# cockroachdb/pebble

Measured on AMD Instinct MI355X. Metric: raw-block GiB/s decoded to KV arrays (device-resident), 1/2/4/8 MI355X, higher is better.
Workload: dtype u8; 1 GPU; config2: 65536 x 32 KiB row-format blocks per GPU, restart interval 16, 16 B keys / 100 B values; blocks_per_gpu=65536, input_bytes_per_gpu=2143748096, kvs_per_gpu=17760256, global_batch_blocks=65536, parallelism=shard1

## Files before the change

### pebble_amd/csrc/common.hip.h

```cpp
#pragma once
#include <hip/hip_runtime.h>
#include <stdint.h>

#include <type_traits>

#include "../../include/pebble_amd.h"

namespace pbl {

typedef uint32_t u32x4 __attribute__((ext_vector_type(4)));
typedef uint32_t u32x2 __attribute__((ext_vector_type(2)));

constexpr int kTPB = 256;
constexpr int kWave = 64;
constexpr int kNumComp = 4;
#ifndef PBL_LB_WIN
#define PBL_LB_WIN 2
#endif
constexpr int kLbWin = PBL_LB_WIN;
#ifndef PBL_LB_L2
#define PBL_LB_L2 0
#endif
constexpr bool kLbL2 = PBL_LB_L2 != 0;

constexpr uint64_t kKindInvalidTrailer = 191u;

__device__ __forceinline__ uint64_t with_seq(uint64_t tr, uint64_t seq, uint32_t flags) {
  return (seq && !(flags & PBL_ROW_RAW_KEYS) && tr != kKindInvalidTrailer) ? (seq << 8) | (tr & 0xff) : tr;
}

constexpr uint64_t kWsHeader = 256;
constexpr int kWsColTick = 2;
constexpr int kWsRowCount = 3;
constexpr uint32_t kSplitChunk = 4096;
constexpr int kStShift = 61;
constexpr uint64_t kStAgg = 1ull << kStShift;
constexpr uint64_t kStWide = 2ull << kStShift;
constexpr uint64_t kStPfx = 3ull << kStShift;
constexpr uint64_t kStPfxWide = 4ull << kStShift;
constexpr uint64_t kStMask = 7ull << kStShift;
constexpr uint64_t kValMask = (1ull << kStShift) - 1;
constexpr int kPkBits[kNumComp] = {14, 18, 18, 11};
constexpr int kPkShift[kNumComp] = {0, 14, 32, 50};
constexpr int kPfBits[kNumComp] = {31, 30, 37, 24};

constexpr uint32_t kL2Chunk = 64;
__host__ __device__ inline uint64_t ws_l2_offset(uint32_t n_blocks) {
  return kWsHeader + uint64_t(2 + 2 * kNumComp) * n_blocks * 8ull;
}
__host__ __device__ inline uint64_t ws_bytes(uint32_t n_blocks) {
  return ws_l2_offset(n_blocks) + 16ull * ((uint64_t(n_blocks) + kL2Chunk - 1) / kL2Chunk);
}
__host__ __device__ inline uint64_t ws_rcnt_offset(uint32_t n_blocks) {
  return ws_l2_offset(n_blocks) - 8ull * (n_blocks + 1);
}
#ifdef PBL_STAMPS
constexpr uint64_t kStampWords = 16;
#else
constexpr uint64_t kStampWords = 0;
#endif
__host__ __device__ inline uint64_t ws_ids_offset(uint32_t n_blocks) {
  return ws_bytes(n_blocks) + kStampWords * 8ull * n_blocks;
}
__host__ __device__ inline uint64_t ws_redo_offset(uint32_t n_blocks) {
  return ws_ids_offset(n_blocks) + 4ull * n_blocks + 4ull * (n_blocks / kSplitChunk + 1) + 8;
}
__host__ __device__ inline uint64_t ws_pend_offset(uint32_t n_blocks) { return ws_redo_offset(n_blocks) + 4ull * n_blocks; }
constexpr uint32_t kEntRec = 64;
__host__ __device__ inline uint64_t ws_ent_offset(uint32_t n_blocks) {
  return (ws_pend_offset(n_blocks) + 4ull * n_blocks + 15) & ~uint64_t(15);
}
__host__ __device__ inline uint64_t ws_alloc_bytes(uint32_t n_blocks) {
  return ws_ent_offset(n_blocks) + 2ull * kEntRec * n_blocks;
}
constexpr uint32_t kLongKeyWgs = PBL_LONGKEY_WGS;
__host__ __device__ inline uint64_t ws_spill_slot_bytes(uint64_t workspace_bytes, uint32_t n_blocks) {
  const uint64_t a = ws_alloc_bytes(n_blocks);
  return workspace_bytes > a ? ((workspace_bytes - a) / kLongKeyWgs) & ~uint64_t(15) : 0;
}


template <class T>
using gptr = __attribute__((address_space(1))) T*;
template <class T>
using lptr = __attribute__((address_space(3))) T*;
template <class T>
__device__ __forceinline__ gptr<T> to_glb(T* p) {
  return (gptr<T>)p;
}
template <class T>
__device__ __forceinline__ lptr<T> to_lds_ptr(T* p) {
  return (lptr<T>)p;
}

__device__ inline uint32_t g_atomic_add(uint32_t* p, uint32_t v) {
  return __hip_atomic_fetch_add(to_glb(p), v, __ATOMIC_RELAXED, __HIP_MEMORY_SCOPE_AGENT);
}
__device__ inline uint32_t g_atomic_or(uint32_t* p, uint32_t v) {
  return __hip_atomic_fetch_or(to_glb(p), v, __ATOMIC_RELAXED, __HIP_MEMORY_SCOPE_AGENT);
}

struct TicketQueue {
  uint32_t* tick;
  uint32_t n_blocks;
  __device__ uint32_t take() const {
    const uint32_t t = g_atomic_add(tick, 1u);
    return t < n_blocks ? t : n_blocks;
  }
};
struct ListQueue {
  uint32_t* tick;
  const uint32_t* ids;
  uint32_t n;
  uint32_t n_blocks;
  __device__ uint32_t take() const {
    const uint32_t t = g_atomic_add(tick, 1u);
    return t < n ? to_glb(ids)[t] : n_blocks;
  }
};

__device__ inline uint64_t ld_agent(const uint64_t* p) {
  return __hip_atomic_load(to_glb(p), __ATOMIC_RELAXED, __HIP_MEMORY_SCOPE_AGENT);
}
__device__ inline void st_agent(uint64_t* p, uint64_t v) {
  __hip_atomic_store(to_glb(p), v, __ATOMIC_RELAXED, __HIP_MEMORY_SCOPE_AGENT);
}

__device__ inline int lane_id() { return threadIdx.x & (kWave - 1); }
__device__ inline int wave_id() { return threadIdx.x >> 6; }

__device__ inline void wave_sync() {
  __builtin_amdgcn_fence(__ATOMIC_RELEASE, "wavefront");
  __builtin_amdgcn_wave_barrier();
  __builtin_amdgcn_fence(__ATOMIC_ACQUIRE, "wavefront");
}

template <typename T>
__device__ inline T wave_incl_scan(T v) {
  const int l = lane_id();
#pragma unroll
  for (int d = 1; d < kWave; d <<= 1) {
    T o = __shfl_up(v, d, kWave);
    if (l >= d) v += o;
  }
  return v;
}
template <typename T>
__device__ inline T wave_sum(T v) {
#pragma unroll
  for (int d = 32; d >= 1; d >>= 1) v += __shfl_xor(v, d, kWave);
  return v;
}

__device__ inline void block_excl_scan2(uint32_t a, uint32_t b, uint32_t* ea, uint32_t* eb,
                                        uint32_t* scratch, uint32_t* tot_a, uint32_t* tot_b) {
  uint32_t ia = wave_incl_scan(a), ib = wave_incl_scan(b);
  const int w = wave_id(), l = lane_id();
  if (l == kWave - 1) { scratch[w] = ia; scratch[4 + w] = ib; }
  __syncthreads();
  uint32_t pa = 0, pb = 0, ta = 0, tb = 0;
#pragma unroll
  for (int i = 0; i < kTPB / kWave; i++) {
    uint32_t sa = scratch[i], sb = scratch[4 + i];
    if (i < w) { pa += sa; pb += sb; }
    ta += sa; tb += sb;
  }
  *ea = pa + ia - a;
  *eb = pb + ib - b;
  *tot_a = ta;
  *tot_b = tb;
}

__device__ inline void lds_stage16(lptr<u32x4> dst, gptr<const u32x4> src, uint32_t n16) {
  const uint32_t l = lane_id();
  for (uint32_t g0 = 0; g0 < n16; g0 += kWave) {
    if (g0 + l < n16)
      __builtin_amdgcn_global_load_lds((gptr<const void>)(src + (g0 + l)), (lptr<void>)(dst + g0), 16, 0, 0);
  }
  asm volatile("s_waitcnt vmcnt(0)" ::: "memory");
  wave_sync();
}

__device__ inline bool agg_packable(const uint64_t agg[kNumComp]) {
  return agg[0] < (1ull << kPkBits[0]) && agg[1] < (1ull << kPkBits[1]) && agg[2] < (1ull << kPkBits[2]) &&
         agg[3] < (1ull << kPkBits[3]);
}
__device__ inline bool pfx_packable(const uint64_t p[kNumComp]) {
  return p[0] < (1ull << kPfBits[0]) && p[1] < (1ull << kPfBits[1]) && p[2] < (1ull << kPfBits[2]) &&
         p[3] < (1ull << kPfBits[3]);
}

struct LbPtrs {
  uint64_t* rec;
  uint64_t* pfx;
  uint64_t* wide;
  uint64_t* l2;
  __device__ LbPtrs(uint64_t* st, uint32_t n_blocks)
      : rec(st), pfx(st + 2ull * n_blocks), wide(st + 2ull * n_blocks + uint64_t(kNumComp) * n_blocks),
        l2(st + (ws_l2_offset(n_blocks) - kWsHeader) / 8) {}
};

__device__ inline void l2_store(const LbPtrs& P, uint32_t chunk, uint64_t tag, const uint64_t p[kNumComp]) {
  st_agent(P.l2 + 2ull * chunk + 1, tag | p[2] | (p[3] << kPfBits[2]));
  st_agent(P.l2 + 2ull * chunk, tag | p[0] | (p[1] << kPfBits[0]));
}

#ifdef PBL_STAMPS
struct LbDiag {
  uint32_t trips, recs, recs2;
  uint64_t poll;
};
#define LBDIAG(...) __VA_ARGS__
#else
struct LbDiag {};
#define LBDIAG(...)
#endif

__device__ inline void lb_store_pfx(const LbPtrs& P, uint32_t n_blocks, uint32_t v, const uint64_t p[kNumComp]) {
  const int l = lane_id();
  if (pfx_packable(p)) {
    if (l == 0) {
      st_agent(P.rec + 2ull * v + 1, kStPfx | p[2] | (p[3] << kPfBits[2]));
      st_agent(P.rec + 2ull * v, kStPfx | p[0] | (p[1] << kPfBits[0]));
    }
  } else {
    if (l < kNumComp) {
      const uint64_t x = l == 0 ? p[0] : l == 1 ? p[1] : l == 2 ? p[2] : p[3];
      st_agent(P.pfx + uint64_t(l) * n_blocks + v, kStPfxWide | (x & kValMask));
    }
    if (l == 0) st_agent(P.rec + 2ull * v, kStPfxWide);
  }
}

__device__ inline void lb_publish(uint64_t* st, uint32_t n_blocks, uint32_t v, const uint64_t agg[kNumComp]) {
  const int l = lane_id();
  const LbPtrs P(st, n_blocks);
  if (v == 0) {
    lb_store_pfx(P, n_blocks, v, agg);
    return;
  }
  if (agg_packable(agg)) {
    if (l == 0) {
      uint64_t packed = 0;
      for (int c = 0; c < kNumComp; c++) packed |= agg[c] << kPkShift[c];
      st_agent(P.rec + 2ull * v, kStAgg | packed);
    }
  } else {
    if (l < kNumComp) {
      const uint64_t a = l == 0 ? agg[0] : l == 1 ? agg[1] : l == 2 ? agg[2] : agg[3];
      st_agent(P.wide + uint64_t(l) * n_blocks + v, kStWide | (a & kValMask));
    }
    if (l == 0) st_agent(P.rec + 2ull * v, kStWide);
  }
}

__device__ inline uint64_t lb_poll(uint64_t* p, uint64_t want, uint32_t* spins, bool* timed_out) {
  uint64_t x;
  while (((x = ld_agent(p)) & kStMask) != want) {
    if (++*spins > (1u << 22)) { *timed_out = true; return 0; }
    __builtin_amdgcn_s_sleep(2);
  }
  return x & kValMask;
}

__device__ inline void lb_fetch4(uint64_t* src, uint32_t n_blocks, int64_t idx, uint64_t want, uint64_t c[kNumComp],
                                 uint32_t* spins, bool* timed_out) {
  uint64_t x[kNumComp];
#pragma unroll
  for (int q = 0; q < kNumComp; q++) x[q] = ld_agent(src + uint64_t(q) * n_blocks + idx);
#pragma unroll
  for (int q = 0; q < kNumComp; q++)
    c[q] = (x[q] & kStMask) == want ? (x[q] & kValMask)
                                    : lb_poll(src + uint64_t(q) * n_blocks + idx, want, spins, timed_out);
}

template <bool L2>
struct LbChunkWin {};
template <>
struct LbChunkWin<true> {
  uint64_t c0, c1;
};
template <int W, bool L2 = false>
struct LbWindows : LbChunkWin<L2> {
  static_assert(!L2 || W >= 2, "two windows reach the chunk edge");
  uint64_t w0[W], w1[W];
  int64_t top;
  __device__ inline int64_t chunk() const { return (top + 1) >> 6; }
  __device__ inline void issue(const LbPtrs& P, int64_t top_) {
    top = top_;
    const int l = lane_id();
    int64_t lo = 0;
    if constexpr (L2) lo = chunk() >= 1 ? (chunk() - 1) * int64_t(kL2Chunk) : 0;
#pragma unroll
    for (int k = 0; k < W; k++) {
      const int64_t idx = top - kWave * k - l;
      const bool in = idx >= lo;
      w0[k] = in ? ld_agent(P.rec + 2 * idx) : idx < 0 ? kStPfx : kStAgg;
      w1[k] = in ? ld_agent(P.rec + 2 * idx + 1) : kStPfx;
    }
    if constexpr (L2) {
      const int64_t c = chunk() - 2 - l;
      this->c0 = c >= 0 ? ld_agent(P.l2 + 2 * c) : kStPfx;
      this->c1 = c >= 0 ? ld_agent(P.l2 + 2 * c + 1) : kStPfx;
    }
  }
};

template <int W, bool L2>
__device__ inline bool lb_consume(const LbPtrs& P, uint32_t n_blocks, const LbWindows<W, L2>& G, uint64_t acc[kNumComp],
                                  int64_t* next_top, int64_t* wait_idx, uint32_t* spins, bool* timed_out, LbDiag* D) {
  const int l = lane_id();
  int64_t top = G.top;
  *wait_idx = -1;
#pragma unroll
  for (int k = 0; k < W; k++) {
    const int64_t idx = G.top - kWave * k - l;
    const uint64_t state = G.w0[k] & kStMask;
    const bool is_pfx = state == kStPfx || state == kStPfxWide;
    const uint64_t pfxm = __ballot(is_pfx);
    const uint64_t notready = __ballot(state == 0);
    const int first = pfxm ? __builtin_ctzll(pfxm) : 64;
    const uint64_t need = first >= 63 ? ~0ull : ((2ull << first) - 1);
    if (notready & need) {
      *wait_idx = G.top - kWave * k - __builtin_ctzll(notready & need);
      *next_top = top;
      return false;
    }
    LBDIAG(D->recs += __builtin_popcountll(__ballot(l <= first && idx >= 0 && (G.w0[k] != kStAgg))));
    uint64_t c[kNumComp] = {0, 0, 0, 0};
    if (l < first && state == kStAgg) {
#pragma unroll
      for (int q = 0; q < kNumComp; q++) c[q] = (G.w0[k] >> kPkShift[q]) & ((1ull << kPkBits[q]) - 1);
    }
    if (l < first && state == kStWide) lb_fetch4(P.wide, n_blocks, idx, kStWide, c, spins, timed_out);
    if (l == first && idx >= 0) {
      if (state == kStPfx) {
        uint64_t w1 = G.w1[k];
        if ((w1 & kStMask) != kStPfx) w1 = kStPfx | lb_poll(P.rec + 2 * idx + 1, kStPfx, spins, timed_out);
        c[0] = G.w0[k] & ((1ull << kPfBits[0]) - 1);
        c[1] = (G.w0[k] >> kPfBits[0]) & ((1ull << kPfBits[1]) - 1);
        c[2] = w1 & ((1ull << kPfBits[2]) - 1);
        c[3] = (w1 >> kPfBits[2]) & ((1ull << kPfBits[3]) - 1);
      } else {
        lb_fetch4(P.pfx, n_blocks, idx, kStPfxWide, c, spins, timed_out);
      }
    }
#pragma unroll
    for (int q = 0; q < kNumComp; q++) acc[q] += c[q];
    if (first < 64) return true;
    top -= kWave;
  }
  if constexpr (L2) {
    const int64_t ck = G.chunk();
    if (ck >= 2) {
      const uint64_t s0 = G.c0 & kStMask, s1 = G.c1 & kStMask;
      const bool there = s0 == s1 && (s0 == kStAgg || s0 == kStPfx);
      const uint64_t pfxm = __ballot(there && s0 == kStPfx), absent = __ballot(!there);
      const int firstp = pfxm ? __builtin_ctzll(pfxm) : 64, firsta = absent ? __builtin_ctzll(absent) : 64;
      const bool ends = firstp < firsta;
      if (ends ? l <= firstp : l < firsta) {
        acc[0] += G.c0 & ((1ull << kPfBits[0]) - 1);
        acc[1] += (G.c0 >> kPfBits[0]) & ((1ull << kPfBits[1]) - 1);
        acc[2] += G.c1 & ((1ull << kPfBits[2]) - 1);
        acc[3] += (G.c1 >> kPfBits[2]) & ((1ull << kPfBits[3]) - 1);
      }
      LBDIAG(D->recs2 += ends ? firstp + (ck - 2 - firstp >= 0) : firsta);
      if (ends) return true;
      top = (ck - 2 - firsta) * int64_t(kL2Chunk) + (kL2Chunk - 1);
    }
  }
  *next_top = top;
  return false;
}

template <int W, bool L2, int WL = W>
__device__ inline void lb_finish(uint64_t* st, uint32_t n_blocks, uint32_t v, const uint64_t agg[kNumComp],
                                 uint64_t excl[kNumComp], uint32_t* timeout_flag, const LbWindows<W, L2>& first_win,
                                 LbDiag* D = nullptr) {
  const int l = lane_id();
  const LbPtrs P(st, n_blocks);
  uint64_t acc[kNumComp] = {0, 0, 0, 0};
  uint32_t spins = 0;
  bool timed_out = false;
  int64_t top = int64_t(v) - 1, wait_idx = -1;
  LBDIAG(LbDiag d0{0, 0, 0, 0}; if (!D) D = &d0; D->trips = v > 0; D->recs = D->recs2 = 0; D->poll = 0);
  if constexpr (L2) {
    if ((v & (kL2Chunk - 1)) == kL2Chunk - 1 && agg_packable(agg)) {
      const uint64_t w = first_win.w0[0];
      if (!__ballot(l < int(kL2Chunk) - 1 && (w & kStMask) != kStAgg)) {
        const uint64_t m = l < int(kL2Chunk) - 1 ? w : 0;
        uint64_t s01 = ((m >> kPkShift[0]) & ((1ull << kPkBits[0]) - 1)) | ((m >> kPkShift[1]) & ((1ull << kPkBits[1]) - 1)) << 32;
        uint64_t s23 = ((m >> kPkShift[2]) & ((1ull << kPkBits[2]) - 1)) | ((m >> kPkShift[3]) & ((1ull << kPkBits[3]) - 1)) << 32;
        s01 = wave_sum(s01);
        s23 = wave_sum(s23);
        const uint64_t ca[kNumComp] = {(s01 & 0xffffffffu) + agg[0], (s01 >> 32) + agg[1], (s23 & 0xffffffffu) + agg[2],
                                       (s23 >> 32) + agg[3]};
        if (l == 0) l2_store(P, v / kL2Chunk, kStAgg, ca);
      }
    }
  }
  bool done = v == 0 || lb_consume(P, n_blocks, first_win, acc, &top, &wait_idx, &spins, &timed_out, D);
  if (__ballot(timed_out)) timed_out = true;
  while (!done && !timed_out) {
    if (wait_idx >= 0) {
      LBDIAG(const uint64_t tp = __builtin_amdgcn_s_memtime());
      if (l == 0) {
        while ((ld_agent(P.rec + 2 * wait_idx) & kStMask) == 0) {
          if (++spins > (1u << 22)) { timed_out = true; break; }
          __builtin_amdgcn_s_sleep(2);
        }
      }
      if (__shfl(timed_out ? 1 : 0, 0, kWave)) { timed_out = true; break; }
      LBDIAG(D->poll += __builtin_amdgcn_s_memtime() - tp);
    }
    LbWindows<WL, L2> G;
    G.issue(P, top);
    LBDIAG(D->trips++);
    done = lb_consume(P, n_blocks, G, acc, &top, &wait_idx, &spins, &timed_out, D);
    if (__ballot(timed_out)) timed_out = true;
  }
  if (timed_out && l == 0) g_atomic_or(timeout_flag, 1u << PBL_TIMEOUT);
#pragma unroll
  for (int q = 0; q < kNumComp; q++) excl[q] = wave_sum(acc[q]);
  if (v > 0) {
    uint64_t p[kNumComp];
#pragma unroll
    for (int q = 0; q < kNumComp; q++) p[q] = excl[q] + agg[q];
    lb_store_pfx(P, n_blocks, v, p);
    if constexpr (L2) {
      if ((v & (kL2Chunk - 1)) == kL2Chunk - 1 && !timed_out && pfx_packable(p) && l == 0)
        l2_store(P, v / kL2Chunk, kStPfx, p);
    }
  }
}

template <int W = kLbWin, bool L2 = false>
__device__ inline void lb_resolve(uint64_t* st, uint32_t n_blocks, uint32_t v, const uint64_t agg[kNumComp],
                                  uint64_t excl[kNumComp], uint32_t* timeout_flag) {
  LbWindows<W, L2> G;
  if (v > 0) G.issue(LbPtrs(st, n_blocks), int64_t(v) - 1);
  lb_finish(st, n_blocks, v, agg, excl, timeout_flag, G);
}

template <bool L2 = false>
__device__ inline void lookback(uint64_t* st, uint32_t n_blocks, uint32_t v, const uint64_t agg[kNumComp],
                                uint64_t excl[kNumComp], uint32_t* timeout_flag) {
  lb_publish(st, n_blocks, v, agg);
  lb_resolve<kLbWin, L2>(st, n_blocks, v, agg, excl, timeout_flag);
}

struct Args {
  pbl_block_batch in;
  pbl_decode_out out;
};

__device__ __forceinline__ uint4 funnel16(const uint4& x, const uint4& y, uint32_t sh) {
  const uint32_t s = sh & 3;
  uint32_t d0, d1, d2, d3, d4;
  switch (sh >> 2) {
    case 0: d0 = x.x; d1 = x.y; d2 = x.z; d3 = x.w; d4 = y.x; break;
    case 1: d0 = x.y; d1 = x.z; d2 = x.w; d3 = y.x; d4 = y.y; break;
    case 2: d0 = x.z; d1 = x.w; d2 = y.x; d3 = y.y; d4 = y.z; break;
    default: d0 = x.w; d1 = y.x; d2 = y.y; d3 = y.z; d4 = y.w; break;
  }
  return make_uint4(__builtin_amdgcn_alignbyte(d1, d0, s), __builtin_amdgcn_alignbyte(d2, d1, s),
                    __builtin_amdgcn_alignbyte(d3, d2, s), __builtin_amdgcn_alignbyte(d4, d3, s));
}

#ifndef PBL_STORE16_NT
#define PBL_STORE16_NT 1
#endif
__device__ inline void store16(uint8_t* base_, uint64_t ga, uint64_t lo, uint64_t hi, uint4 w) {
  const gptr<uint8_t> base = to_glb(base_);
  if (ga >= lo && ga + 16 <= hi) {
#if PBL_STORE16_NT
    __builtin_nontemporal_store(u32x4{w.x, w.y, w.z, w.w}, (gptr<u32x4>)(base + ga));
#else
    *(gptr<u32x4>)(base + ga) = u32x4{w.x, w.y, w.z, w.w};
#endif
    return;
  }
#pragma unroll
  for (int i = 0; i < 16; i++) {
    uint32_t word = i < 4 ? w.x : i < 8 ? w.y : i < 12 ? w.z : w.w;
    if (ga + i >= lo && ga + i < hi) base[ga + i] = uint8_t(word >> (8 * (i & 3)));
  }
}

typedef u32x4 u32x4_u __attribute__((aligned(1)));
typedef uint64_t u64_u __attribute__((aligned(1)));
typedef uint32_t u32_u __attribute__((aligned(1)));
typedef uint16_t u16_u __attribute__((aligned(1)));
__device__ __forceinline__ void copy_chunks(gptr<uint8_t> dst, gptr<const uint8_t> src, uint32_t n) {
  uint32_t c = 0;
  for (; c + 64 <= n; c += 64) {
    u32x4 x[4];
#pragma unroll
    for (int u = 0; u < 4; u++) x[u] = *(gptr<const u32x4_u>)(src + c + 16 * u);
#pragma unroll
    for (int u = 0; u < 4; u++) *(gptr<u32x4_u>)(dst + c + 16 * u) = x[u];
  }
  for (; c + 16 <= n; c += 16) *(gptr<u32x4_u>)(dst + c) = *(gptr<const u32x4_u>)(src + c);
  if (c < n) {
    const u32x4 w = *(gptr<const u32x4_u>)(src + c);
    const uint32_t r = n - c;
    uint64_t lo = uint64_t(w.x) | uint64_t(w.y) << 32, hi = uint64_t(w.z) | uint64_t(w.w) << 32;
    uint32_t o = c;
    if (r & 8) {
      *(gptr<u64_u>)(dst + o) = lo;
      lo = hi;
      o += 8;
    }
    if (r & 4) {
      *(gptr<u32_u>)(dst + o) = uint32_t(lo);
      lo >>= 32;
      o += 4;
    }
    if (r & 2) {
      *(gptr<u16_u>)(dst + o) = uint16_t(lo);
      lo >>= 16;
      o += 2;
    }
    if (r & 1) dst[o] = uint8_t(lo);
  }
}

__device__ inline void write_block_meta(const pbl_decode_out& O, uint32_t b, uint32_t nb, uint32_t status,
                                        const uint64_t excl[kNumComp], const uint64_t agg[kNumComp],
                                        bool slow) {
  to_glb(O.blk_kv_base)[b] = excl[0];
  to_glb(O.blk_key_base)[b] = excl[1];
// ... 39 lines not shown
```

### pebble_amd/csrc/rowblk_pool.hip.h

```cpp
#pragma once

#include "rowblk_core.hip.h"
#include "rowblk_general.hip.h"
#include "rowblk_big.hip.h"

namespace pbl {
namespace row {
namespace pool {

#ifndef PBL_POOL_WAVES
#define PBL_POOL_WAVES 8
#endif
#ifndef PBL_POOL_STAGES
#define PBL_POOL_STAGES 3
#endif
#ifndef PBL_POOL_SLEEP
#define PBL_POOL_SLEEP 8
#endif
#ifndef PBL_POOL_PRIO
#define PBL_POOL_PRIO 2
#endif
#ifndef PBL_POOL_EARLYREL
#define PBL_POOL_EARLYREL 2
#endif
#ifndef PBL_POOL_PREFETCH
#define PBL_POOL_PREFETCH 0
#endif
#ifndef PBL_POOL_PREFETCH_LATE
#define PBL_POOL_PREFETCH_LATE 1
#endif
#ifndef PBL_POOL_LB_WIN
#define PBL_POOL_LB_WIN PBL_LB_WIN
#endif
#ifndef PBL_POOL_LB_WIN_LATER
#define PBL_POOL_LB_WIN_LATER 1
#endif
constexpr int kPoolLbWin = PBL_POOL_LB_WIN;
constexpr int kPoolLbWinLater = kLbL2 ? kPoolLbWin : PBL_POOL_LB_WIN_LATER;
constexpr int kEarlyRel = PBL_POOL_EARLYREL;
constexpr uint32_t kPrefetch = PBL_POOL_PREFETCH;
constexpr int kNW = PBL_POOL_WAVES;
constexpr int kNS = PBL_POOL_STAGES;
constexpr int kTPBP = kNW * kWave;
constexpr uint32_t kMaxKl = 4095;

struct Stage {
  uint4 x[kLdsBlkBytes / 16];
};

__device__ __forceinline__ uint32_t m_ksrc(uint64_t m) { return uint32_t(m) & 0x7fffu; }
__device__ __forceinline__ uint32_t m_sh(uint64_t m) { return uint32_t(m >> 15) & 0xfffu; }
__device__ __forceinline__ uint32_t m_klen(uint64_t m) { return uint32_t(m >> 27) & 0xfffu; }
__device__ __forceinline__ uint32_t m_par(uint64_t m) { return uint32_t(m >> 39) & 0x1ffu; }
__device__ __forceinline__ uint32_t m_hl(uint64_t m) { return uint32_t(m >> 48) & 0xfu; }
__device__ __forceinline__ uint32_t m_fl(uint64_t m) { return uint32_t(m >> 52) & 0xffu; }
__device__ __forceinline__ uint64_t m_pack(uint32_t ksrc, uint32_t sh, uint32_t kl, uint32_t par, uint32_t hl,
                                           uint32_t fl) {
  return uint64_t(ksrc) | uint64_t(sh) << 15 | uint64_t(kl) << 27 | uint64_t(par) << 39 | uint64_t(hl) << 48 |
         uint64_t(fl) << 52;
}

constexpr int kPerSlot = (163840 - kNS * int(sizeof(Stage)) - 256) / kNW;
template <bool kHide>
constexpr int slot_kv() {
  const int n = ((kPerSlot - 32) / (kHide ? 14 : 12)) & ~7;
  return n > 511 ? 511 : n;
}
template <bool kHide>
struct Slot {
  static constexpr int kKv = slot_kv<kHide>();
  uint64_t m0[kKv];
  uint32_t vp[kKv + 5];
  uint16_t ent[kHide ? kKv : 1];
};

template <bool kHide>
struct PoolLds {
  Stage st[kNS];
  Slot<kHide> sl[kNW];
  uint32_t free_mask;
};
static_assert(sizeof(PoolLds<true>) <= 163840 && sizeof(PoolLds<false>) <= 163840, "one pool workgroup per CU");

typedef u32x4 u32x4_ug __attribute__((aligned(1)));
typedef uint32_t u32_ug __attribute__((aligned(1)));
typedef uint64_t u64_ug __attribute__((aligned(1)));
typedef uint16_t u16_ug __attribute__((aligned(1)));

__device__ __forceinline__ uint32_t dpp_incl_scan(uint32_t v) {
  v += __builtin_amdgcn_update_dpp(0u, v, 0x111, 0xf, 0xf, false);
  v += __builtin_amdgcn_update_dpp(0u, v, 0x112, 0xf, 0xf, false);
  v += __builtin_amdgcn_update_dpp(0u, v, 0x114, 0xf, 0xf, false);
  v += __builtin_amdgcn_update_dpp(0u, v, 0x118, 0xf, 0xf, false);
  v += __builtin_amdgcn_update_dpp(0u, v, 0x142, 0xa, 0xf, false);
  v += __builtin_amdgcn_update_dpp(0u, v, 0x143, 0xc, 0xf, false);
  return v;
}
__device__ __forceinline__ uint32_t last_lane(uint32_t v) { return __builtin_amdgcn_readlane(v, kWave - 1); }

#ifndef PBL_POOL_NT
#define PBL_POOL_NT 1
#endif
template <class T>
__device__ __forceinline__ void st_out(gptr<T> p, T v) {
#if PBL_POOL_NT
  __builtin_nontemporal_store(v, p);
#else
  *p = v;
#endif
}

#ifndef PBL_POOL_SBASE
#define PBL_POOL_SBASE 0
#endif
#ifndef PBL_POOL_VFAST
#define PBL_POOL_VFAST 1
#endif
constexpr bool kSBase = PBL_POOL_SBASE != 0;
constexpr bool kVFast = PBL_POOL_VFAST != 0;
// ... 767 lines not shown
      }
    }
  }
}

template <bool kHide>
__device__ __forceinline__ uint32_t acquire(PoolLds<kHide>& L) {
  uint32_t s = 0;
  if (lane_id() == 0) {
    for (;;) {
      const uint32_t m = __hip_atomic_load(&L.free_mask, __ATOMIC_RELAXED, __HIP_MEMORY_SCOPE_WORKGROUP);
      if (m) {
        const uint32_t c = uint32_t(__builtin_ctz(m));
        const uint32_t old =
            __hip_atomic_fetch_and(&L.free_mask, ~(1u << c), __ATOMIC_ACQUIRE, __HIP_MEMORY_SCOPE_WORKGROUP);
        if (old & (1u << c)) {
          s = c;
          break;
        }
      } else {
        __builtin_amdgcn_s_sleep(PBL_POOL_SLEEP);
      }
    }
  }
  if (PBL_POOL_PRIO) __builtin_amdgcn_s_setprio(PBL_POOL_PRIO);
  return __builtin_amdgcn_readfirstlane(__shfl(s, 0, kWave));
}

template <bool kHide>
__device__ __forceinline__ int32_t try_acquire(PoolLds<kHide>& L) {
  int32_t s = -1;
  if (lane_id() == 0) {
    const uint32_t m = __hip_atomic_load(&L.free_mask, __ATOMIC_RELAXED, __HIP_MEMORY_SCOPE_WORKGROUP);
    if (m) {
      const uint32_t c = uint32_t(__builtin_ctz(m));
      const uint32_t old =
          __hip_atomic_fetch_and(&L.free_mask, ~(1u << c), __ATOMIC_ACQUIRE, __HIP_MEMORY_SCOPE_WORKGROUP);
      if (old & (1u << c)) s = int32_t(c);
    }
  }
  return __builtin_amdgcn_readfirstlane(__shfl(s, 0, kWave));
}

template <bool kHide>
__device__ __forceinline__ void release(PoolLds<kHide>& L, uint32_t s, bool drop_prio = true) {
  asm volatile("s_waitcnt lgkmcnt(0)" ::: "memory");
  wave_sync();
  if (lane_id() == 0) __hip_atomic_fetch_or(&L.free_mask, 1u << s, __ATOMIC_RELEASE, __HIP_MEMORY_SCOPE_WORKGROUP);
  if (PBL_POOL_PRIO && drop_prio) __builtin_amdgcn_s_setprio(0);
}

__device__ __forceinline__ void stage_dma(Stage& S, const uint8_t* blocks, uint64_t boff, uint32_t blen) {
  const int l = lane_id();
  const uint64_t a0 = boff & ~uint64_t(15), a1 = (boff + blen + 15) & ~uint64_t(15);
  const uint32_t n16 = uint32_t((a1 - a0) >> 4);
  const gptr<const uint8_t> base = to_glb(blocks + a0);
  for (uint32_t g0 = 0; g0 < n16; g0 += kWave) {
    if (g0 + l < n16)
      __builtin_amdgcn_global_load_lds((gptr<const void>)(base + 16ull * (g0 + l)),
                                       (lptr<void>)to_lds_ptr(reinterpret_cast<void*>(&S.x[1 + g0])), 16, 0, 0);
  }
}

__device__ __noinline__ void block_slow(Stage& S, uint8_t* keybuf, uint32_t keycap, const Args A, uint32_t b,
                                        uint64_t boff, uint32_t blen) {
  const int l = lane_id();
  const uint32_t nb = A.in.n_blocks, flags = A.in.flags;
  const pbl_decode_out& O = A.out;
  uint64_t* lb_state = reinterpret_cast<uint64_t*>(reinterpret_cast<uint8_t*>(O.workspace) + kWsHeader);
  SlowState ss;
  uint64_t dummy[kNumComp] = {0, 0, 0, 0}, excl[kNumComp];
  const uint8_t* src = reinterpret_cast<const uint8_t*>(S.x) + kPad + (boff & 15);
  bool from_lds = true;
  slow_walk(src, true, blen, flags, A.in.synthetic_seq_num, keybuf, keycap, kPassCount, O, b, dummy, &ss);
  if (ss.status == PBL_UNSUPPORTED) {
    from_lds = false;
    src = A.in.blocks + boff;
    keybuf = reinterpret_cast<uint8_t*>(S.x);
    keycap = uint32_t(kLdsBlkBytes);
    slow_walk(src, false, blen, flags, A.in.synthetic_seq_num, keybuf, keycap, kPassCount, O, b, dummy, &ss);
  }
  const bool okk = ss.status == PBL_OK;
  const uint64_t agg[kNumComp] = {okk ? ss.nkv : 0, okk ? ss.kb : 0, okk ? ss.vb : 0, okk ? ss.nr : 0};
  lookback<kLbL2>(lb_state, nb, b, agg, excl, &O.totals->status_mask);
  uint32_t st2 = ss.status;
  if (okk && overflows(O, excl, agg)) st2 = PBL_OVERFLOW;
  if (st2 == PBL_OK) slow_walk(src, from_lds, blen, flags, A.in.synthetic_seq_num, keybuf, keycap, kPassAll, O, b, excl, &ss);
  else if (l == 0 && O.key_off && excl[0] + b < O.kv_cap + nb) {
    to_glb(O.key_off)[excl[0] + b] = 0;
    to_glb(O.val_off)[excl[0] + b] = 0;
  }
  if (l == 0) write_block_meta(O, b, nb, st2, excl, agg, true);
}

__device__ __noinline__ void block_big(const Args A, uint32_t b, uint64_t boff, uint32_t blen, uint8_t* keybuf,
                                       uint32_t keycap) {
  const int l = lane_id();
  const uint32_t nb = A.in.n_blocks;
  const pbl_decode_out& O = A.out;
  uint64_t* lb_state = reinterpret_cast<uint64_t*>(reinterpret_cast<uint8_t*>(O.workspace) + kWsHeader);
  const uint32_t st0 = to_glb(O.blk_status)[b];
  const bool okk = st0 == PBL_OK;
  const uint64_t agg[kNumComp] = {okk ? to_glb(O.blk_kv_base)[b] : 0, okk ? to_glb(O.blk_key_base)[b] : 0,
                                  okk ? to_glb(O.blk_val_base)[b] : 0,
                                  okk ? uint64_t(GlbBlk{to_glb(A.in.blocks + boff), blen}.le32(blen - 4)) : 0};
  uint64_t excl[kNumComp];
  lb_resolve<kLbWin, kLbL2>(lb_state, nb, b, agg, excl, &O.totals->status_mask);
  uint32_t st2 = st0;
  if (okk && overflows(O, excl, agg)) st2 = PBL_OVERFLOW;
  if (l == 0) {
    if (st2 != PBL_OK && O.key_off && excl[0] + b < O.kv_cap + nb) {
      to_glb(O.key_off)[excl[0] + b] = 0;
      to_glb(O.val_off)[excl[0] + b] = 0;
    }
    write_block_meta(O, b, nb, st2, excl, agg, true);
  }
  if (st2 == PBL_OK) {
    SlowState ss;
    slow_walk_t<GlbBlk, PBL_BIG_U>(GlbBlk{to_glb(A.in.blocks + boff), blen}, blen, A.in.flags,
                                    A.in.synthetic_seq_num, to_lds_ptr(keybuf), keycap, kPassAll, O, b, excl, &ss);
    if (ss.status == PBL_UNSUPPORTED && l == 0) {
      uint32_t* hdr = reinterpret_cast<uint32_t*>(O.workspace);
      uint32_t* pend = reinterpret_cast<uint32_t*>(reinterpret_cast<uint8_t*>(O.workspace) + ws_pend_offset(nb));
      to_glb(pend)[g_atomic_add(hdr + rowc::kWsBigPend, 1u)] = b;
    } else if (ss.status != PBL_OK && l == 0) {
      to_glb(O.blk_status)[b] = ss.status;
      g_atomic_or(&O.totals->status_mask, 1u << ss.status);
      g_atomic_add(&O.totals->n_bad_blocks, 1u);
    }
  }
}

struct Pend {
  uint64_t boff;
  uint32_t b, status, nkv, tkb, tvb, nres, roff, blen;
  bool live;
};

template <bool kHide>
__device__ __forceinline__ Pend block_front(PoolLds<kHide>& L, uint32_t s, uint32_t b, uint64_t boff, uint32_t blen,
                                            bool staged, Slot<kHide>& W, const Args& A) {
  Stage& S = L.st[s];
  const int l = lane_id();
  const uint32_t nb = A.in.n_blocks, flags = A.in.flags;
  const bool vprefix = (flags & PBL_ROW_VALUE_PREFIX) && !(flags & PBL_ROW_RAW_KEYS);
  uint64_t* lb_state = reinterpret_cast<uint64_t*>(reinterpret_cast<uint8_t*>(A.out.workspace) + kWsHeader);
  constexpr uint32_t kKv = uint32_t(Slot<kHide>::kKv);
  Pend P;
  P.b = b;
  P.boff = boff;
  P.blen = blen;
  P.live = false;
  P.nkv = P.tkb = P.tvb = P.nres = P.roff = 0;
  P.status = PBL_OK;

  if (blen > kMaxFastLen) {
    release(L, s);
    block_big(A, b, boff, blen, reinterpret_cast<uint8_t*>(&W), uint32_t(sizeof(W)));
    return P;
  }
  PSTAMP(A, b, 1, l == 0);
  if (!staged) stage_dma(S, A.in.blocks, boff, blen);
  asm volatile("s_waitcnt vmcnt(0)" ::: "memory");
  wave_sync();
  PSTAMP(A, b, 2, l == 0);
  const View V = lds_view(S.x, uint32_t(kPad + (boff & 15)));
  uint32_t roff, nres;
  uint32_t status = init_checks(LdsBlk{V}, blen, flags, &roff, &nres);
  bool slow = status == PBL_OK && nres > kKv;
  uint32_t nkv = 0, tkb = 0, tvb = 0;
  bool published = false, released = false;
  if (status == PBL_OK && !slow && roff > 0) {
    const uint32_t R = (nres + kWave - 1) / kWave;
    const uint32_t r0 = min(uint32_t(l) * R, nres), r1 = min(r0 + R, nres);
    PAcc acc{0, 0, 0, 0};
    bool ok = true, bad = false, vbad = false, over = false;
    PRun RB;
    RB.n = 0;
    RB.pos = RB.e0 = RB.prev_kl = RB.prev_kind = RB.rw = 0;
    const bool single = R == 1;
    walk_runs<kHide>(V, r0, r1, nres, roff, flags, vprefix, single, RB, acc, ok, bad, vbad, over);
    const uint32_t ic = dpp_incl_scan(acc.cnt), ik = dpp_incl_scan(acc.kb), iv = dpp_incl_scan(acc.vb);
    const uint32_t ie = kHide ? dpp_incl_scan(acc.ne) : ic;
    nkv = last_lane(ic);
    tkb = last_lane(ik);
    tvb = last_lane(iv);
    const uint32_t nent = kHide ? last_lane(ie) : nkv;
    if (__ballot(bad)) status = PBL_CORRUPT_BOUNDS;
    else if (__ballot(!ok) || nent > kKv) slow = true;
    else if (__ballot(vbad)) status = PBL_CORRUPT_BOUNDS;
// ... 4 lines not shown
      PSTAMP(A, b, 3, l == 0);
      if (kEarlyRel && single && !vprefix && !__ballot(over)) {
        release(L, s, kEarlyRel != 2);
        released = true;
        PSTAMP(A, b, 9, l == 0);
      }
      MState M{ie - (kHide ? acc.ne : acc.cnt), ic - acc.cnt, iv - acc.vb, 0, 0, 0};
      meta_runs<kHide>(W, V, r0, r1, nres, roff, flags, vprefix, single, over, RB, M);
      if (l < 5) W.vp[nkv + l] = tvb;
      PSTAMP(A, b, 4, l == 0);
    }
  }
  if (status == PBL_OK && slow) {
    block_slow(S, reinterpret_cast<uint8_t*>(W.m0), uint32_t(sizeof(W.m0)), A, b, boff, blen);
    release(L, s);
    PSTAMP(A, b, 9, l == 0);
    return P;
  }
  if (!released) {
    release(L, s);
    PSTAMP(A, b, 9, l == 0);
  } else if (PBL_POOL_PRIO && kEarlyRel == 2) {
    __builtin_amdgcn_s_setprio(0);
  }
  if (!published) {
    const bool okb = status == PBL_OK;
    const uint64_t agg[kNumComp] = {okb ? nkv : 0, okb ? tkb : 0, okb ? tvb : 0, okb ? nres : 0};
    lb_publish(lb_state, nb, b, agg);
    if (l < 5) W.vp[l] = 0;
  }
  P.status = status;
  P.nkv = status == PBL_OK ? nkv : 0;
  P.tkb = status == PBL_OK ? tkb : 0;
  P.tvb = status == PBL_OK ? tvb : 0;
  P.nres = status == PBL_OK ? nres : 0;
  P.roff = roff;
  P.live = true;
  return P;
}

struct Next {
  uint32_t t, w;
};
constexpr uint32_t kNextHave = 4, kNextStaged = 8, kNextDone = 16;
static_assert(kNS <= 4, "Next::w keeps the stage in two bits");

template <bool kHide>
__device__ __forceinline__ void prefetch(PoolLds<kHide>& L, const Args& A, const uint32_t* ids, uint32_t nt, Next& X) {
  const int32_t s = try_acquire(L);
  if (s < 0) return;
  uint32_t t = 0;
  if (lane_id() == 0) t = g_atomic_add(reinterpret_cast<uint32_t*>(A.out.workspace), 1u);
  t = __builtin_amdgcn_readfirstlane(__shfl(t, 0, kWave));
  if (t >= nt) {
    release(L, uint32_t(s));
    X.w = kNextDone;
    return;
  }
  if (ids) t = __builtin_amdgcn_readfirstlane(to_glb(ids)[t]);
  const uint64_t boff = to_glb(A.in.block_off)[t];
  const uint32_t blen = to_glb(A.in.block_len)[t];
  const bool staged = blen <= kMaxFastLen;
  X.t = t;
  X.w = uint32_t(s) | kNextHave | (staged ? kNextStaged : 0u);
  if (staged) stage_dma(L.st[s], A.in.blocks, boff, blen);
  PSTAMP(A, t, 10, lane_id() == 0);
}

template <bool kHide>
__device__ __forceinline__ void block_emit(const Pend& P, const Slot<kHide>& W, const Args& A, PoolLds<kHide>& L,
                                           const uint32_t* ids, uint32_t nt, Next& X) {
  const int l = lane_id();
  const uint32_t nb = A.in.n_blocks, flags = A.in.flags, b = P.b;
  const pbl_decode_out& O = A.out;
  uint64_t* lb_state = reinterpret_cast<uint64_t*>(reinterpret_cast<uint8_t*>(O.workspace) + kWsHeader);
  const uint8_t* gblk = A.in.blocks + P.boff;
  const gptr<const uint8_t> gb = ubase<kSBase>(to_glb(gblk));
  const uint32_t ph = uint32_t(uint64_t(gblk) & 15u);
  const gptr<const uint8_t> g16 = ubase<kSBase>(to_glb(gblk - ph));
  constexpr bool kFastSteps = kVFast && kUni && kVDepth == 1;
  const GSrc KS{gb, P.blen, uint32_t(((uint64_t(gblk) + P.blen + 15) & ~uint64_t(15)) - uint64_t(gblk))};
  const bool raw = (flags & PBL_ROW_RAW_KEYS) != 0;
  const uint32_t nkv = P.nkv, nres = P.nres;
  LbWindows<kPoolLbWin, kLbL2> G;
  if (b > 0) G.issue(LbPtrs(lb_state, nb), int64_t(b) - 1);
  KBatch K;
  VBatch VB, VB1;
  VDesc VD{0, 0, true};
  uint32_t rs0 = 0;
  const bool ok0 = P.status == PBL_OK;
  if (ok0) {
    key_load<kHide, GSrc>(W, KS, raw, 0, nkv, K);
    if (kFastSteps) VD = val_desc(W.vp, nkv, 0);
    if (kFastSteps && VD.fast) val_load_fast(g16, ph, VD.lw, VB);
    else val_load(W.vp, gb, nkv, 0, VB);
    if (kVDepth == 2) val_load(W.vp, gb, nkv, 8 * kVG, VB1);
    if (O.restarts && uint32_t(l) < nres) rs0 = KS.le32(P.roff + 4 * l);
  }
  const uint64_t agg[kNumComp] = {nkv, P.tkb, P.tvb, nres};
  uint64_t excl[kNumComp];
#ifdef PBL_STAMPS
  LbDiag LD;
  lb_finish<kPoolLbWin, kLbL2, kPoolLbWinLater>(lb_state, nb, b, agg, excl, &O.totals->status_mask, G, &LD);
  if (l == 0) {
    uint64_t* sp = reinterpret_cast<uint64_t*>(reinterpret_cast<uint8_t*>(O.workspace) + ws_bytes(nb)) + uint64_t(b) * 16;
    sp[11] = LD.trips;
    sp[12] = LD.recs;
    sp[13] = LD.poll;
    sp[14] = LD.recs2;
  }
#else
  lb_finish<kPoolLbWin, kLbL2, kPoolLbWinLater>(lb_state, nb, b, agg, excl, &O.totals->status_mask, G);
#endif
  PSTAMP(A, b, 5, l == 0);
  uint32_t status = P.status;
  if (ok0 && overflows(O, excl, agg)) status = PBL_OVERFLOW;
  if (l == 0) {
    if (status != PBL_OK && O.key_off && excl[0] + b < O.kv_cap + nb) {
      to_glb(O.key_off)[excl[0] + b] = 0;
      to_glb(O.val_off)[excl[0] + b] = 0;
    }
    write_block_meta(O, b, nb, status, excl, agg, false);
  }
  if (status != PBL_OK) return;

  const uint64_t kvb = uni64<kSBase>(excl[0]), kbb = uni64<kSBase>(excl[1]), vbb = uni64<kSBase>(excl[2]),
                 rbb = uni64<kSBase>(excl[3]);
  const gptr<uint32_t> p_rst = ubase<kSBase>(to_glb(O.restarts) + rbb);
  if (O.restarts && uint32_t(l) < nres) p_rst[uint32_t(l)] = rs0;
  uint32_t kcar = 0;
  const gptr<uint8_t> vbytes = ubase<kSBase>(to_glb(O.val_bytes) + vbb);
  if (kUni) {
    bool pf = kPrefetch != 0;
    if (kFastSteps) {
      for (uint32_t j0 = 0; j0 <= nkv; j0 += kWave) {
        KBatch KN;
        VBatch VN;
        VDesc DN{0, 0, true};
        const bool more = j0 + kWave <= nkv;
        if (pf && (nkv - j0) / kWave + PBL_POOL_PREFETCH_LATE <= kPrefetch) {
          prefetch<kHide>(L, A, ids, nt, X);
          pf = false;
        }
        if (more) {
          DN = val_desc(W.vp, nkv, j0 + kWave);
          if (DN.fast) val_load_fast(g16, ph, DN.lw, VN);
          else val_load(W.vp, gb, nkv, j0 + kWave, VN);
          key_load<kHide, GSrc>(W, KS, raw, j0 + kWave, nkv, KN);
        }
        key_store<kHide, GSrc, 0, true, true>(W, KS, A, b, j0, nkv, kvb, kbb, K, kcar, VD.sw & 0xffffu);
        if (VD.fast) val_store_fast(VD.sw, VB, vbytes);
        else val_store(W.vp, nkv, j0, VB, gb, vbytes);
        K = KN;
        VB = VN;
        VD = DN;
      }
    } else if (kVDepth == 1) {
      for (uint32_t j0 = 0; j0 <= nkv; j0 += kWave) {
        KBatch KN;
        VBatch VN;
        const bool more = j0 + kWave <= nkv;
        if (pf && (nkv - j0) / kWave + PBL_POOL_PREFETCH_LATE <= kPrefetch) {
          prefetch<kHide>(L, A, ids, nt, X);
          pf = false;
        }
        if (more) {
          key_load<kHide, GSrc>(W, KS, raw, j0 + kWave, nkv, KN);
          val_load(W.vp, gb, nkv, j0 + kWave, VN);
        }
        key_store<kHide, GSrc, 0, true>(W, KS, A, b, j0, nkv, kvb, kbb, K, kcar);
        val_store(W.vp, nkv, j0, VB, gb, vbytes);
        K = KN;
        VB = VN;
      }
    } else {
      for (uint32_t j0 = 0; j0 <= nkv; j0 += kWave) {
        KBatch KN;
        VBatch VN;
        if (pf && (nkv - j0) / kWave + PBL_POOL_PREFETCH_LATE <= kPrefetch) {
          prefetch<kHide>(L, A, ids, nt, X);
          pf = false;
        }
        if (j0 + kWave <= nkv) key_load<kHide, GSrc>(W, KS, raw, j0 + kWave, nkv, KN);
        if (j0 + 2 * kWave < nkv) val_load(W.vp, gb, nkv, j0 + 2 * kWave, VN);
        key_store<kHide, GSrc>(W, KS, A, b, j0, nkv, kvb, kbb, K, kcar);
        val_store(W.vp, nkv, j0, VB, gb, vbytes);
        K = KN;
        VB = VB1;
        VB1 = VN;
      }
    }
    if (O.restarts)
      for (uint32_t r = kWave + l; r < nres; r += kWave) p_rst[r] = KS.le32(P.roff + 4 * r);
    copy_long_values(W.vp, gb, nkv, vbytes);
    PSTAMP(A, b, 6, l == 0);
// ... 69 lines not shown
```

Before: 1512 GiB/s.

## Use 16-byte buffer loads/stores and partial-lane windows in decoupled lookback

The lookback record reads and the packed prefix publish now use single 128-bit buffer load/store instructions instead of two separate 64-bit agent-scope accesses, so each record is seen atomically and takes fewer memory ops. Later lookback trips in the pool emit path also alternate between a 16-lane partial window and a full-wave window, which shortens each poll round when the predecessor is close. This is meant to cut latency on the serial scan chain between blocks. It relies on 16-byte aligned record storage and the buffer-resource bounds being right, and the narrower windows may need more trips when the prefix lies far back.

```diff
diff --git a/pebble_amd/csrc/common.hip.h b/pebble_amd/csrc/common.hip.h
--- a/pebble_amd/csrc/common.hip.h
+++ b/pebble_amd/csrc/common.hip.h
@@ -30,6 +30,7 @@
 }
 
 constexpr uint64_t kWsHeader = 256;
+static_assert(kWsHeader % 16 == 0, "rec[] is read and written 16 bytes at a time");
 constexpr int kWsColTick = 2;
 constexpr int kWsRowCount = 3;
 constexpr uint32_t kSplitChunk = 4096;
@@ -190,6 +191,19 @@
          p[3] < (1ull << kPfBits[3]);
 }
 
+constexpr int kLbV16 = 1;
+constexpr int kLbSt16 = 2;
+
+__device__ __forceinline__ __amdgpu_buffer_rsrc_t lb_rsrc(const uint64_t* p, uint32_t bytes) {
+  const uint64_t a = reinterpret_cast<uint64_t>(p);
+  const uint32_t alo = uint32_t(__builtin_amdgcn_readfirstlane(uint32_t(a)));
+  const uint32_t ahi = uint32_t(__builtin_amdgcn_readfirstlane(uint32_t(a >> 32)));
+  const uint64_t u = uint64_t(alo) | uint64_t(ahi) << 32;
+  return __builtin_amdgcn_make_buffer_rsrc(reinterpret_cast<void*>(u), 0, __builtin_amdgcn_readfirstlane(bytes),
+                                           0x00020000);
+}
+constexpr int kAuxSc1 = 16;
+
 struct LbPtrs {
   uint64_t* rec;
   uint64_t* pfx;
@@ -216,12 +230,19 @@
 #define LBDIAG(...)
 #endif
 
+template <int F = 0>
 __device__ inline void lb_store_pfx(const LbPtrs& P, uint32_t n_blocks, uint32_t v, const uint64_t p[kNumComp]) {
   const int l = lane_id();
   if (pfx_packable(p)) {
     if (l == 0) {
-      st_agent(P.rec + 2ull * v + 1, kStPfx | p[2] | (p[3] << kPfBits[2]));
-      st_agent(P.rec + 2ull * v, kStPfx | p[0] | (p[1] << kPfBits[0]));
+      if constexpr (F & kLbSt16) {
+        const uint64_t x0 = kStPfx | p[0] | (p[1] << kPfBits[0]), x1 = kStPfx | p[2] | (p[3] << kPfBits[2]);
+        const u32x4 x = {uint32_t(x0), uint32_t(x0 >> 32), uint32_t(x1), uint32_t(x1 >> 32)};
+        __builtin_amdgcn_raw_buffer_store_b128(x, lb_rsrc(P.rec + 2ull * v, 16), 0, 0, kAuxSc1);
+      } else {
+        st_agent(P.rec + 2ull * v + 1, kStPfx | p[2] | (p[3] << kPfBits[2]));
+        st_agent(P.rec + 2ull * v, kStPfx | p[0] | (p[1] << kPfBits[0]));
+      }
     }
   } else {
     if (l < kNumComp) {
@@ -280,23 +301,40 @@
 struct LbChunkWin<true> {
   uint64_t c0, c1;
 };
-template <int W, bool L2 = false>
+template <int W, bool L2 = false, int F = 0>
 struct LbWindows : LbChunkWin<L2> {
   static_assert(!L2 || W >= 2, "two windows reach the chunk edge");
   uint64_t w0[W], w1[W];
   int64_t top;
+  int lanes;
   __device__ inline int64_t chunk() const { return (top + 1) >> 6; }
-  __device__ inline void issue(const LbPtrs& P, int64_t top_) {
+  __device__ inline void issue(const LbPtrs& P, int64_t top_, int lanes_ = kWave) {
     top = top_;
+    lanes = lanes_;
     const int l = lane_id();
     int64_t lo = 0;
     if constexpr (L2) lo = chunk() >= 1 ? (chunk() - 1) * int64_t(kL2Chunk) : 0;
-#pragma unroll
-    for (int k = 0; k < W; k++) {
-      const int64_t idx = top - kWave * k - l;
-      const bool in = idx >= lo;
-      w0[k] = in ? ld_agent(P.rec + 2 * idx) : idx < 0 ? kStPfx : kStAgg;
-      w1[k] = in ? ld_agent(P.rec + 2 * idx + 1) : kStPfx;
+    if constexpr (F & kLbV16) {
+      const int64_t low = top - int64_t(kWave) * W + 1, base = low > lo ? low : lo;
+      const __amdgpu_buffer_rsrc_t rs = lb_rsrc(P.rec + 2 * base, uint32_t(top - base + 1) * 16u);
+#pragma unroll
+      for (int k = 0; k < W; k++) {
+        const int64_t idx = top - kWave * k - l;
+        const bool in = idx >= lo && l < lanes;
+        const uint64_t o0 = idx < 0 && l < lanes ? kStPfx : kStAgg;
+        u32x4 x = {uint32_t(o0), uint32_t(o0 >> 32), 0u, uint32_t(kStPfx >> 32)};
+        if (in) x = __builtin_amdgcn_raw_buffer_load_b128(rs, uint32_t(idx - base) * 16u, 0, kAuxSc1);
+        w0[k] = x[0] | uint64_t(x[1]) << 32;
+        w1[k] = x[2] | uint64_t(x[3]) << 32;
+      }
+    } else {
+#pragma unroll
+      for (int k = 0; k < W; k++) {
+        const int64_t idx = top - kWave * k - l;
+        const bool in = idx >= lo && l < lanes;
+        w0[k] = in ? ld_agent(P.rec + 2 * idx) : idx < 0 && l < lanes ? kStPfx : kStAgg;
+        w1[k] = in ? ld_agent(P.rec + 2 * idx + 1) : kStPfx;
+      }
     }
     if constexpr (L2) {
       const int64_t c = chunk() - 2 - l;
@@ -306,8 +344,8 @@
   }
 };
 
-template <int W, bool L2>
-__device__ inline bool lb_consume(const LbPtrs& P, uint32_t n_blocks, const LbWindows<W, L2>& G, uint64_t acc[kNumComp],
+template <int W, bool L2, int F>
+__device__ inline bool lb_consume(const LbPtrs& P, uint32_t n_blocks, const LbWindows<W, L2, F>& G, uint64_t acc[kNumComp],
                                   int64_t* next_top, int64_t* wait_idx, uint32_t* spins, bool* timed_out, LbDiag* D) {
   const int l = lane_id();
   int64_t top = G.top;
@@ -348,7 +386,7 @@
 #pragma unroll
     for (int q = 0; q < kNumComp; q++) acc[q] += c[q];
     if (first < 64) return true;
-    top -= kWave;
+    top -= W == 1 ? G.lanes : kWave;
   }
   if constexpr (L2) {
     const int64_t ck = G.chunk();
@@ -373,10 +411,11 @@
   return false;
 }
 
-template <int W, bool L2, int WL = W>
+template <int W, bool L2, int WL = W, int F = 0, int LL = kWave>
 __device__ inline void lb_finish(uint64_t* st, uint32_t n_blocks, uint32_t v, const uint64_t agg[kNumComp],
-                                 uint64_t excl[kNumComp], uint32_t* timeout_flag, const LbWindows<W, L2>& first_win,
+                                 uint64_t excl[kNumComp], uint32_t* timeout_flag, const LbWindows<W, L2, F>& first_win,
                                  LbDiag* D = nullptr) {
+  static_assert(LL == kWave || (WL == 1 && !L2 && LL > 0 && LL < kWave), "a partial trip is one window of the one-level form");
   const int l = lane_id();
   const LbPtrs P(st, n_blocks);
   uint64_t acc[kNumComp] = {0, 0, 0, 0};
@@ -401,6 +440,7 @@
   }
   bool done = v == 0 || lb_consume(P, n_blocks, first_win, acc, &top, &wait_idx, &spins, &timed_out, D);
   if (__ballot(timed_out)) timed_out = true;
+  bool part = LL < kWave;
   while (!done && !timed_out) {
     if (wait_idx >= 0) {
       LBDIAG(const uint64_t tp = __builtin_amdgcn_s_memtime());
@@ -413,11 +453,16 @@
       if (__shfl(timed_out ? 1 : 0, 0, kWave)) { timed_out = true; break; }
       LBDIAG(D->poll += __builtin_amdgcn_s_memtime() - tp);
     }
-    LbWindows<WL, L2> G;
-    G.issue(P, top);
+    LbWindows<WL, L2, F> G;
+    if constexpr (LL < kWave) {
+      G.issue(P, top, part ? LL : kWave);
+    } else {
+      G.issue(P, top);
+    }
     LBDIAG(D->trips++);
     done = lb_consume(P, n_blocks, G, acc, &top, &wait_idx, &spins, &timed_out, D);
     if (__ballot(timed_out)) timed_out = true;
+    if (LL < kWave && wait_idx < 0) part = !part;
   }
   if (timed_out && l == 0) g_atomic_or(timeout_flag, 1u << PBL_TIMEOUT);
 #pragma unroll
@@ -426,7 +471,7 @@
     uint64_t p[kNumComp];
 #pragma unroll
     for (int q = 0; q < kNumComp; q++) p[q] = excl[q] + agg[q];
-    lb_store_pfx(P, n_blocks, v, p);
+    lb_store_pfx<F>(P, n_blocks, v, p);
     if constexpr (L2) {
       if ((v & (kL2Chunk - 1)) == kL2Chunk - 1 && !timed_out && pfx_packable(p) && l == 0)
         l2_store(P, v / kL2Chunk, kStPfx, p);
@@ -434,19 +479,19 @@
   }
 }
 
-template <int W = kLbWin, bool L2 = false>
+template <int W = kLbWin, bool L2 = false, int F = 0>
 __device__ inline void lb_resolve(uint64_t* st, uint32_t n_blocks, uint32_t v, const uint64_t agg[kNumComp],
                                   uint64_t excl[kNumComp], uint32_t* timeout_flag) {
-  LbWindows<W, L2> G;
+  LbWindows<W, L2, F> G;
   if (v > 0) G.issue(LbPtrs(st, n_blocks), int64_t(v) - 1);
-  lb_finish(st, n_blocks, v, agg, excl, timeout_flag, G);
-}
-
-template <bool L2 = false>
+  lb_finish<W, L2, W, F>(st, n_blocks, v, agg, excl, timeout_flag, G);
+}
+
+template <bool L2 = false, int F = 0>
 __device__ inline void lookback(uint64_t* st, uint32_t n_blocks, uint32_t v, const uint64_t agg[kNumComp],
                                 uint64_t excl[kNumComp], uint32_t* timeout_flag) {
   lb_publish(st, n_blocks, v, agg);
-  lb_resolve<kLbWin, L2>(st, n_blocks, v, agg, excl, timeout_flag);
+  lb_resolve<kLbWin, L2, F>(st, n_blocks, v, agg, excl, timeout_flag);
 }
 
 struct Args {
diff --git a/pebble_amd/csrc/rowblk_pool.hip.h b/pebble_amd/csrc/rowblk_pool.hip.h
--- a/pebble_amd/csrc/rowblk_pool.hip.h
+++ b/pebble_amd/csrc/rowblk_pool.hip.h
@@ -35,6 +35,17 @@
 #ifndef PBL_POOL_LB_WIN_LATER
 #define PBL_POOL_LB_WIN_LATER 1
 #endif
+#ifndef PBL_LB_V16
+#define PBL_LB_V16 1
+#endif
+#ifndef PBL_POOL_LB_ST16
+#define PBL_POOL_LB_ST16 1
+#endif
+#ifndef PBL_POOL_LB_LATER_LANES
+#define PBL_POOL_LB_LATER_LANES 16
+#endif
+constexpr int kPoolLbF = (PBL_LB_V16 ? kLbV16 : 0) | (PBL_POOL_LB_ST16 ? kLbSt16 : 0);
+constexpr int kPoolLbLaterLanes = kLbL2 ? kWave : PBL_POOL_LB_LATER_LANES;
 constexpr int kPoolLbWin = PBL_POOL_LB_WIN;
 constexpr int kPoolLbWinLater = kLbL2 ? kPoolLbWin : PBL_POOL_LB_WIN_LATER;
 constexpr int kEarlyRel = PBL_POOL_EARLYREL;
@@ -968,7 +979,7 @@
   }
   const bool okk = ss.status == PBL_OK;
   const uint64_t agg[kNumComp] = {okk ? ss.nkv : 0, okk ? ss.kb : 0, okk ? ss.vb : 0, okk ? ss.nr : 0};
-  lookback<kLbL2>(lb_state, nb, b, agg, excl, &O.totals->status_mask);
+  lookback<kLbL2, kPoolLbF>(lb_state, nb, b, agg, excl, &O.totals->status_mask);
   uint32_t st2 = ss.status;
   if (okk && overflows(O, excl, agg)) st2 = PBL_OVERFLOW;
   if (st2 == PBL_OK) slow_walk(src, from_lds, blen, flags, A.in.synthetic_seq_num, keybuf, keycap, kPassAll, O, b, excl, &ss);
@@ -991,7 +1002,7 @@
                                   okk ? to_glb(O.blk_val_base)[b] : 0,
                                   okk ? uint64_t(GlbBlk{to_glb(A.in.blocks + boff), blen}.le32(blen - 4)) : 0};
   uint64_t excl[kNumComp];
-  lb_resolve<kLbWin, kLbL2>(lb_state, nb, b, agg, excl, &O.totals->status_mask);
+  lb_resolve<kLbWin, kLbL2, kPoolLbF>(lb_state, nb, b, agg, excl, &O.totals->status_mask);
   uint32_t st2 = st0;
   if (okk && overflows(O, excl, agg)) st2 = PBL_OVERFLOW;
   if (l == 0) {
@@ -1162,7 +1173,7 @@
   const GSrc KS{gb, P.blen, uint32_t(((uint64_t(gblk) + P.blen + 15) & ~uint64_t(15)) - uint64_t(gblk))};
   const bool raw = (flags & PBL_ROW_RAW_KEYS) != 0;
   const uint32_t nkv = P.nkv, nres = P.nres;
-  LbWindows<kPoolLbWin, kLbL2> G;
+  LbWindows<kPoolLbWin, kLbL2, kPoolLbF> G;
   if (b > 0) G.issue(LbPtrs(lb_state, nb), int64_t(b) - 1);
   KBatch K;
   VBatch VB, VB1;
@@ -1181,7 +1192,7 @@
   uint64_t excl[kNumComp];
 #ifdef PBL_STAMPS
   LbDiag LD;
-  lb_finish<kPoolLbWin, kLbL2, kPoolLbWinLater>(lb_state, nb, b, agg, excl, &O.totals->status_mask, G, &LD);
+  lb_finish<kPoolLbWin, kLbL2, kPoolLbWinLater, kPoolLbF, kPoolLbLaterLanes>(lb_state, nb, b, agg, excl, &O.totals->status_mask, G, &LD);
   if (l == 0) {
     uint64_t* sp = reinterpret_cast<uint64_t*>(reinterpret_cast<uint8_t*>(O.workspace) + ws_bytes(nb)) + uint64_t(b) * 16;
     sp[11] = LD.trips;
@@ -1190,7 +1201,7 @@
     sp[14] = LD.recs2;
   }
 #else
-  lb_finish<kPoolLbWin, kLbL2, kPoolLbWinLater>(lb_state, nb, b, agg, excl, &O.totals->status_mask, G);
+  lb_finish<kPoolLbWin, kLbL2, kPoolLbWinLater, kPoolLbF, kPoolLbLaterLanes>(lb_state, nb, b, agg, excl, &O.totals->status_mask, G);
 #endif
   PSTAMP(A, b, 5, l == 0);
   uint32_t status = P.status;
```

Measured after the change: 1698 GiB/s, median of 6. +12.3%, better.
